# GRIPS-code/pyLBL

Measured on AMD Instinct MI355X. Metric: line×gridpoint Voigt evals/sec (whole job; per GPU: evals_per_s_per_gpu; spectra/sec: spectra_per_s), higher is better.
Workload: dtype f64; 1 GPU; BASELINE config 'target': 1 level(s) per GPU, H2O+CO2, grid 1-5000 cm-1 at 0.001 cm-1 (5000000 points), cut_off 25, remove_pedestal=False; levels_total=1, atmosphere=surface, output=gas, parallelism=levels sharded

## Files before the change

include/lbl_amd.h:

```cpp
#ifndef LBL_AMD_H_
#define LBL_AMD_H_

#include <stdint.h>

#ifdef __cplusplus
extern "C" {
#endif

#define LBL_OK              0
#define LBL_ERROR           1
#define LBL_BAD_ARGUMENT    2
#define LBL_NO_DEVICE       3
#define LBL_OUT_OF_RANGE    4
#define LBL_TABLE_OPEN_FAILED       10
#define LBL_TABLE_NO_ALIAS          11
#define LBL_TABLE_NO_TIPS           12
#define LBL_TABLE_NOT_RECTANGULAR   13
#define LBL_TABLE_NO_ISOTOPOLOGUES  14
#define LBL_TABLE_NO_TRANSITIONS    15

#define LBL_RANGE_REFERENCE 0
#define LBL_RANGE_SKIP      1

#define LBL_PREP_DEVICE     0
// ... 214 lines not shown
                     int32_t flags, double *out, int64_t level_stride);

int lbl_xsec_bands(lbl_engine *engine, int32_t xsec, double temperature, double pressure,
                   double *values);

int lbl_absorption(double pressure, double temperature, double volume_mixing_ratio,
                   int v0, int vn, int n_per_v, double *k, char *database, char *formula,
                   int cut_off, int remove_pedestal);

#ifndef LBL_NO_REFERENCE_SYMBOL
int absorption(double pressure, double temperature, double volume_mixing_ratio,
               int v0, int vn, int n_per_v, double *k, char *database, char *formula,
               int cut_off, int remove_pedestal);
#endif

typedef struct lbl_table lbl_table;
int lbl_table_read(const char *path, const char *name, lbl_table **table);
int lbl_table_shape(const lbl_table *table, int64_t *n_lines, int32_t *molecule_id,
                    int32_t *n_isotopologues, int32_t *num_iso, int32_t *num_t,
                    char *formula, int32_t formula_bytes);
int lbl_table_copy(const lbl_table *table, double *columns, int32_t *local_iso_id,
                   int64_t *isoid, double *mass, double *tips_temperature, double *tips_data);
int lbl_table_free(lbl_table *table);

int lbl_molecule_load_sqlite(lbl_engine *engine, const char *path, const char *name,
                             int32_t *molecule);

int lbl_compat_state(int32_t *device, int32_t *resident);

const char *lbl_version(void);

int lbl_wing_batches(const int32_t *bounds);

#ifdef __cplusplus
}
#endif
#endif
```

pylbl_amd/csrc/accumulate.h:

```cpp
#pragma once

#include <hip/hip_runtime.h>

#include "line_prep.h"
#include "voigt_profile.h"

namespace lbl {

struct Tiling
{
    int aligned;
    int per_cell;
    int length;
    int n_tiles;
};

__host__ __device__ inline void tile_bounds(const Tiling & t, int tile, int n_per_v, int n,
                                            long long & i0, long long & i1)
{
    if (t.aligned)
    {
        const int cell = tile/t.per_cell;
        const int sub = tile - cell*t.per_cell;
        i0 = (long long)cell*n_per_v + (long long)sub*t.length;
        i1 = i0 + t.length - 1;
        const long long cell_end = (long long)(cell + 1)*n_per_v - 1;
        if (i1 > cell_end) i1 = cell_end;
    }
    else
    {
        i0 = (long long)tile*t.length;
        i1 = i0 + t.length - 1;
    }
    if (i1 > n - 1) i1 = n - 1;
}

struct alignas(32) TileSchedule
{
// ... 5 lines not shown
{
    const double v_lo = (double)v0 + (double)i0*dv;
    const double v_hi = (double)v0 + (double)i1*dv;
    return 0.5*(v_lo + v_hi);
}

#ifndef LBL_WING_GROUP
#define LBL_WING_GROUP 8
#endif
#ifndef LBL_FAR_TERMS
#define LBL_FAR_TERMS 21
#define LBL_FAR_RATIO 4.
#endif
constexpr int kFarTerms = LBL_FAR_TERMS;
constexpr double kFarRatio = LBL_FAR_RATIO;

struct alignas(16) WorkItem
{
    int tile;
    int part, parts;
    int slot;
};

struct AccumulateArgs
{
    const LineWing * wing;
    const LineCore * core;
    const TileSchedule * schedule;
    const LevelScalars * levels;
    const WorkItem * items;
    const double * far_series;
    const int * wing_bounds;
    int wing_batches;
    double * partial;
    long long partial_slots;
    double * k;
    long long level_stride;
    long long n_lines;
    Tiling tiling;
    int n_tiles;
    int n;
    int v0, n_per_v;
    double dv;
    double v0_real;
    int scale_density;
    int accumulate;
    int inner_everywhere;
#ifdef LBL_ABLATE
    int ablate;
#endif
};

#ifdef LBL_ABLATE
#define LBL_ABLATED(a, bits) (((a).ablate & (bits)) != 0)
#else
#define LBL_ABLATED(a, bits) false
#endif

}

#include "accumulate_lines.h"

namespace lbl {

__device__ __forceinline__ void share_of(int j0, int j1, int part, int parts, float inverse,
                                         int unit_shift, int & begin, int & end)
// ... 15 lines not shown
    const int level = blockIdx.y;
    const WorkItem item = a.items[blockIdx.x];
    const int tile = item.tile;
    long long first_point, last_point;
    tile_bounds(a.tiling, tile, a.n_per_v, a.n, first_point, last_point);
    const int i0 = (int)first_point, i1 = (int)last_point;
    const TileSchedule sc = a.schedule[(long long)level*a.n_tiles + tile];
    const LineWing * __restrict__ wing = a.wing + (long long)level*a.n_lines;
    const LineCore * __restrict__ core = a.core + (long long)level*a.n_lines;

    double v[P], acc[P];
    double * slab = &partial[wave][0][0];
    __shared__ InnerStage inner_stage[4];
    const double first_index = (double)(i0 + lane);
#pragma unroll
    for (int p = 0; p < P; ++p)
    {
        const double step = (first_index + (double)(p*64))*a.dv;
        v[p] = a.v0_real + step;
        acc[p] = 0.;
    }

    const int piece = item.part*4 + wave, pieces = item.parts*4;
    GeneralList g;
    int fa0, fa1, fb0, fb1, e;
    const bool clipped_in_groups = !a.inner_everywhere && !LBL_ABLATED(a, 64);
    const float inverse = 1.f/(float)pieces;
    share_of(sc.lo, sc.a1, piece, pieces, inverse, clipped_in_groups ? 3 : 0, g.begin[0], e);
    g.count[0] = e - g.begin[0];
    share_of(sc.c1, sc.c2, piece, pieces, inverse, 0, g.begin[1], e);
    g.count[1] = e - g.begin[1];
    share_of(sc.a2, sc.hi, piece, pieces, inverse, clipped_in_groups ? 3 : 0, g.begin[2], e);
    g.count[2] = e - g.begin[2];
    share_of(sc.f1, sc.c1, piece, pieces, inverse, 2, fa0, fa1);
    share_of(sc.c2, sc.f2, piece, pieces, inverse, 2, fb0, fb1);
    g.begin[3] = fa0 + ((fa1 - fa0) & ~3);
    g.count[3] = (fa1 - fa0) & 3;
    g.begin[4] = fb0 + ((fb1 - fb0) & ~3);
    g.count[4] = (fb1 - fb0) & 3;
    if (LBL_ABLATED(a, 4)) { g.count[0] = 0; g.count[2] = 0; }
    if (LBL_ABLATED(a, 8)) { g.count[3] = 0; g.count[4] = 0; }
    if (LBL_ABLATED(a, 16)) { g.count[1] = 0; }
    if (!LBL_ABLATED(a, 2))
    {
        int batches = 1;
        if (P == 4)
        {
            const int * __restrict__ wb = a.wing_bounds + level*kWingBounds;
            const int bound[kWingBounds] = {wb[0], wb[1], wb[2], wb[3]};
            batches = __builtin_amdgcn_readfirstlane(min(wing_batches(bound), a.wing_batches));
        }
        fast_ranges<P>(wing, fa0, fa1, fb0, fb1, batches, v, acc);
    }
    bool slab_in_use = false;
    if (!LBL_ABLATED(a, 1))
    {
        GeneralList walk = g;
        if (clipped_in_groups)
        {
            clipped_ranges<P>(wing, core, g.begin[0], g.count[0], g.begin[2], g.count[2], i0, i1,
                              lane, v, acc);
            walk.count[0] = walk.count[2] = 0;
        }
        general_ranges<P>(wing, core, walk, i0, i1, lane, v, acc);
        if (!LBL_ABLATED(a, 32) && a.levels[level].inner_possible != 0.)
        {
            GeneralList inner = g;
            if (!a.inner_everywhere)
            {
                inner.count[0] = inner.count[2] = inner.count[3] = inner.count[4] = 0;
            }
            slab_in_use = inner_ranges(wing, core, inner, inner_stage[wave], i0, i1, a.v0,
                                       a.n_per_v, a.dv, lane, slab, P);
        }
    }

#pragma unroll
    for (int p = 0; p < P; ++p)
    {
        partial[wave][p][lane] = slab_in_use ? partial[wave][p][lane] + acc[p] : acc[p];
    }
    __syncthreads();

    const bool add_series = a.far_series != nullptr && item.part == 0;
    const double * __restrict__ series = a.far_series +
// ... 122 lines not shown
```

pylbl_amd/csrc/accumulate_lines.h:

```cpp
#pragma once

namespace lbl {

template <int P>
__device__ __forceinline__ void fast_ranges(const LineWing * __restrict__ wing,
                                            int a0, int a1, int b0, int b1, int batches,
                                            const double (&v)[P], double (&acc)[P])
{
    const int qa = (a1 - a0) >> 2;
    const int quads = qa + ((b1 - b0) >> 2);
    int q = 0;
#if LBL_WING_GROUP == 8
    auto eight = [&](int at, WingTerm (&l)[8]) {
        const int ja = at < qa ? a0 + 4*at : b0 + 4*(at - qa);
        const int jb = (at + 1) < qa ? a0 + 4*(at + 1) : b0 + 4*(at + 1 - qa);
#pragma unroll
        for (int i = 0; i < 4; ++i)
        {
            const LineWing wa = wing[ja + i], wb = wing[jb + i];
            l[i] = WingTerm{wa.centre, wa.g2, wa.bl};
            l[4 + i] = WingTerm{wb.centre, wb.g2, wb.bl};
        }
    };
    if (P == 4 && batches > 1)
    {
        const int eights = quads >> 1;
        for (int o = 0; o < eights; )
        {
            const int stop = min(o + batches, eights);
            double num[P], den[P];
            {
                WingTerm l[8];
                eight(2*o, l);
#pragma unroll
                for (int p = 0; p < P; ++p)
                {
                    wing_eight(v[p], l, num[p], den[p]);
                }
            }
            for (++o; o < stop; ++o)
            {
                WingTerm l[8];
                eight(2*o, l);
#pragma unroll
                for (int p = 0; p < P; ++p)
                {
                    double n, t;
                    wing_eight(v[p], l, n, t);
                    num[p] = __builtin_fma(num[p], t, n*den[p]);
                    den[p] = den[p]*t;
                }
            }
#pragma unroll
            for (int p = 0; p < P; ++p)
            {
                acc[p] = __builtin_fma(num[p], rcp_newton(den[p]), acc[p]);
            }
        }
        q = 2*eights;
    }
    for (; q + 2 <= quads; q += 2)
    {
        WingTerm l[8];
        eight(q, l);
#pragma unroll
        for (int p = 0; p < P; ++p)
        {
            acc[p] = lorentz_eight(v[p], l, acc[p]);
        }
    }
#endif
    for (; q < quads; ++q)
    {
        const int j = q < qa ? a0 + 4*q : b0 + 4*(q - qa);
        const LineWing l1 = wing[j], l2 = wing[j + 1], l3 = wing[j + 2], l4 = wing[j + 3];
#pragma unroll
        for (int p = 0; p < P; ++p)
        {
            acc[p] = lorentz_four(v[p], l1.centre, l1.g2, l1.bl, l2.centre, l2.g2, l2.bl,
                                  l3.centre, l3.g2, l3.bl, l4.centre, l4.g2, l4.bl, acc[p]);
        }
    }
}

__device__ __forceinline__ unsigned row_bits(int lo, int hi, int rows)
{
    lo = max(lo, 0);
    hi = min(hi, rows - 1);
    return lo > hi ? 0u : ((2u << hi) - 1u) & ~((1u << lo) - 1u);
}

__device__ __forceinline__ unsigned rows_meeting(int a, int b, int i0, int rows)
{
    return b < a ? 0u : row_bits((a - i0) >> 6, (b - i0) >> 6, rows);
}

__device__ __forceinline__ unsigned rows_inside(int a, int b, int i0, int rows)
{
    return b < a ? 0u : row_bits((a - i0 + 63) >> 6, (b - 63 - i0) >> 6, rows);
}

template <int P>
__device__ __forceinline__ void general_line(const LineWing & l, const LineCore & c,
                                             int i0, int i1, int lane,
                                             const double (&v)[P], double (&acc)[P])
{
    const unsigned in_window = rows_meeting(l.first, l.last, i0, P);
    if (in_window == 0)
    {
        return;
    }
    const unsigned all_region_one = rows_inside(c.mid_first, c.mid_last, i0, P) &
                                    ~rows_meeting(c.hole_first, c.hole_last, i0, P);
// ... 421 lines not shown
```

pylbl_amd/csrc/compute_stages.inc:

```
namespace {

struct CallShape
{
    Molecule * m = nullptr;
    GridSpec g;
    long long n_long = 0;
    long long stride = 0;
    RangeRule rule;
    Tiling tiling;
    int farfield = 0;
    int points = 0;
};

int shape_of(lbl_engine * engine, const ComputeRequest & rq, CallShape & s)
{
    s.m = find_molecule(engine, rq.molecule);
    if (s.m == nullptr) return fail(engine, LBL_BAD_ARGUMENT, "unknown molecule handle.");
    if (rq.n_levels < 1 || rq.temperature == nullptr || rq.pressure == nullptr ||
        rq.vmr == nullptr)
    {
        return fail(engine, LBL_BAD_ARGUMENT, "need at least one level with T, P and x.");
    }
    if (rq.n_per_v < 1 || rq.vn <= rq.v0 || rq.cut_off < 0)
    {
// ... 159 lines not shown
    bool streamed;
    int pieces;
    bool with_pedestal;
    long long out_bytes;
    long long chunk;
};

void reserve_for_call(const LinesCall & c)
{
    const ComputeRequest & rq = c.rq;
    const CallShape & s = c.shape;
    const CallTraits & t = c.traits;
    Lane & lane = c.lane;
    const long long n_lines = s.m->n_lines, n_tiles = s.tiling.n_tiles, chunk = c.chunk;
    lane.level_feed.refill((size_t)chunk);
    lane.levels.reserve((size_t)chunk);
    lane.wing.reserve((size_t)(chunk*std::max(n_lines, 1ll)));
    lane.core.reserve((size_t)(chunk*std::max(n_lines, 1ll)));
    lane.schedule.reserve((size_t)(chunk*n_tiles));
    if (t.want_k && !t.out_device) lane.staging.reserve((size_t)(chunk*s.n_long));
    if (c.with_pedestal && t.out_device && t.add_into_block)
    {
        lane.raw.reserve((size_t)(chunk*s.n_long));
    }
    if (t.want_k && s.farfield)
    {
        lane.far_series.reserve((size_t)(chunk*n_tiles*kFarTerms));
    }
    if (t.want_k)
    {
        lane.partial.reserve((size_t)std::max(1ll, chunk*c.plan.partial_slots*64*s.points));
    }
    lane.wing_bounds.reserve((size_t)(chunk*kWingBounds));
    if (rq.evals != nullptr)
    {
        lane.evals.reserve(1);
        HIP_TRY(hipMemsetAsync(lane.evals.data, 0, sizeof(unsigned long long), c.stream));
    }
    if (rq.derived != nullptr) lane.derived.reserve((size_t)(std::max(n_lines, 1ll)*8));
}

void launch_far_series(lbl_engine * engine, Lane & lane, const CallShape & s, int count,
                       hipStream_t stream)
{
    const GridSpec & g = s.g;
    const int n_tiles = s.tiling.n_tiles;
    const int n_groups = (n_tiles + kFarGroup - 1)/kFarGroup;
    const long long n_lines = s.m->n_lines;
    engine->timed(kTimeSchedule, stream, [&] {
        dim3 far_grid((unsigned)(((n_groups + 7)/8)*8), (unsigned)count);
        hipLaunchKernelGGL(farfield_series_kernel, far_grid, dim3(256), 0, stream, lane.wing.data,
                           lane.schedule.data, s.m->d_column[0].data, lane.levels.data, n_lines,
                           s.tiling, n_groups, g.v0, g.n_per_v, g.n, g.dv, lane.far_series.data);
        HIP_TRY(hipGetLastError());
    }, 1);
}

void bound_inner_regions(const Molecule & m, const RangeRule & rule, LevelScalars & lv)
{
    lv.inner_possible = 1.;
    const double foreign = lv.p_atm - lv.p_partial;
    if (foreign >= 0. && lv.p_partial >= 0. && m.min_gamma_air >= 0. &&
        m.min_gamma_self >= 0. && m.n_lines > 0)
    {
        double widest = 0.;
        for (int slot = 0; slot < kMassSlots; ++slot)
// ... 30 lines not shown
        {
            return fail(c.engine, LBL_OUT_OF_RANGE,
                        "level " + std::to_string(base + l) + ": " + why);
        }
        bound_inner_regions(*c.shape.m, c.shape.rule, lv);
    }
    if (!levels_inline(c.engine, count))
    {
        lane.level_feed.upload(lane.levels.data, (size_t)count, c.stream);
    }
    return LBL_OK;
}

int inner_points_everywhere(const LevelScalars * levels, int count, const ComputeRequest & rq,
                            const CallShape & s)
{
    double reach = 0.;
    for (int l = 0; l < count; ++l)
    {
        const LevelScalars & lv = levels[l];
        const double kk = lv.core_reach;
        reach = std::max(reach, kk < 0.5 ? kk*(rq.vn + 1.)/(1. - kk) + 2.*lv.shift_max : 1.e9);
    }
    const double tile_width = (double)s.tiling.length*s.g.dv;
    return (rq.cut_off - 1. <= reach + tile_width + 1.) ? 1 : 0;
}

struct HostPrep
{
    std::vector<LineWing> wing;
    std::vector<LineCore> core;
    std::vector<double> derived;
    std::vector<int> wing_bounds;
};

void prepare_on_host(lbl_engine * engine, Lane & lane, const ComputeRequest & rq,
                     const CallShape & s, int count, hipStream_t stream, HostPrep & hp)
{
    const Molecule & m = *s.m;
    const long long n_lines = m.n_lines;
    if (n_lines > 0)
    {
        hp.wing.resize((size_t)(count*n_lines));
        hp.core.resize((size_t)(count*n_lines));
        if (rq.derived != nullptr) hp.derived.assign((size_t)(n_lines*8), 0.);
        hp.wing_bounds.assign((size_t)(count*kWingBounds), kWingBoundsFill);
        unsigned long long total = 0;
        for (int l = 0; l < count; ++l)
        {
            for (long long j = 0; j < n_lines; ++j)
            {
                const bool ok = m.iso_slot[j] >= 0 &&
                                line_accepted(s.rule, m.column[0][j], m.order[j]);
                double * d = (rq.derived != nullptr && l == 0) ? hp.derived.data() + j*8
                                                               : nullptr;
                LineWing & w = hp.wing[(size_t)(l*n_lines + j)];
                const int status = prepare_line(
                    lane.level_feed.block[l], s.g, m.column[0][j], m.column[1][j], m.column[2][j],
                    m.column[3][j], m.column[4][j], m.column[5][j], m.column[6][j],
                    std::max(m.iso_slot[j], 0), ok, w, hp.core[(size_t)(l*n_lines + j)], d);
                if (status == 1 && w.last >= w.first) total += w.last - w.first + 1;
                int bound[kWingBounds];
                wing_line_bounds(s.g, m.column[0][j], status, w,
                                 hp.core[(size_t)(l*n_lines + j)], bound);
                for (int b = 0; b < kWingBounds; ++b)
                {
                    int & least = hp.wing_bounds[(size_t)(l*kWingBounds + b)];
                    least = std::min(least, bound[b]);
                }
            }
        }
        engine->timed(kTimePrepare, stream, [&] {
            HIP_TRY(hipMemcpyAsync(lane.wing.data, hp.wing.data(),
                                   hp.wing.size()*sizeof(LineWing), hipMemcpyHostToDevice,
                                   stream));
            HIP_TRY(hipMemcpyAsync(lane.core.data, hp.core.data(),
                                   hp.core.size()*sizeof(LineCore), hipMemcpyHostToDevice,
                                   stream));
            HIP_TRY(hipMemcpyAsync(lane.wing_bounds.data, hp.wing_bounds.data(),
                                   hp.wing_bounds.size()*sizeof(int), hipMemcpyHostToDevice,
                                   stream));
        });
        HIP_TRY(hipStreamSynchronize(stream));
        if (rq.evals != nullptr) *rq.evals += (int64_t)total;
    }
    if (rq.k != nullptr)
    {
        engine->timed(kTimeSchedule, stream, [&] {
            dim3 grid((unsigned)((8ll*s.tiling.n_tiles + 255)/256), (unsigned)count);
            hipLaunchKernelGGL(schedule_kernel, grid, dim3(256), 0, stream, m.view(),
                               lane.levels.data, s.g, s.tiling, s.farfield, lane.schedule.data);
            HIP_TRY(hipGetLastError());
        });
    }
}

void launch_prologue(const LinesCall & c, int count, HostPrep & hp)
{
    lbl_engine * engine = c.engine;
    const ComputeRequest & rq = c.rq;
    const CallShape & s = c.shape;
    Lane & lane = c.lane;
    hipStream_t stream = c.stream;
    if (engine->prep == LBL_PREP_HOST)
    {
        prepare_on_host(engine, lane, rq, s, count, stream, hp);
        return;
    }
    const bool inline_levels = levels_inline(engine, count);
    InlineLevels packed;
    if (inline_levels)
    {
        std::memcpy(packed.level, lane.level_feed.block, count*sizeof(LevelScalars));
    }
    const int prepare_blocks = (int)((s.m->n_lines + 255)/256);
    const int schedule_blocks = c.traits.want_k ? (int)((8ll*s.tiling.n_tiles + 255)/256) : 0;
    HIP_TRY(hipMemsetAsync(lane.wing_bounds.data, 0x7f, (size_t)count*kWingBounds*sizeof(int),
                           stream));
    engine->timed(kTimePrepare, stream, [&] {
        dim3 grid((unsigned)std::max(prepare_blocks + schedule_blocks, 1), (unsigned)count);
        hipLaunchKernelGGL(prologue_kernel, grid, dim3(256), 0, stream, s.m->view(),
                           lane.levels.data, packed, inline_levels ? 1 : 0, s.g, s.rule, s.tiling,
                           s.farfield, prepare_blocks, lane.wing.data, lane.core.data,
                           lane.schedule.data,
                           rq.derived != nullptr ? lane.derived.data : nullptr,
                           rq.evals != nullptr ? lane.evals.data : nullptr,
                           lane.wing_bounds.data);
        HIP_TRY(hipGetLastError());
    });
}

Lane::Pass pass_of(const LinesCall & c, long long base, int count)
{
    const CallTraits & t = c.traits;
    Lane::Pass p;
    p.base = base;
    p.count = count;
    p.target = t.out_device ? c.rq.k + base*c.shape.stride : c.lane.staging.data;
    p.target_stride = t.out_device ? c.shape.stride : c.shape.n_long;
    p.sums = p.target;
    p.sums_stride = p.target_stride;
    if (c.with_pedestal && t.out_device && t.add_into_block)
    {
        p.sums = c.lane.raw.data;
        p.sums_stride = c.shape.n_long;
    }
    p.ped_stream = c.engine->overlap_pedestal ? c.lane.side : c.stream;
    p.finish_stream = c.with_pedestal ? p.ped_stream : c.stream;
    return p;
}

void start_pedestal_search(const LinesCall & c, const Lane::Pass & p)
{
    lbl_engine * engine = c.engine;
    Lane & lane = c.lane;
    if (engine->overlap_pedestal)
    {
        lane.prepared.record(c.stream);
        HIP_TRY(hipStreamWaitEvent(lane.side, lane.prepared, 0));
    }
    engine->timed(kTimePedestal, p.ped_stream, [&] {
        pedestal_find_runs(lane.pedestal, p.ped_stream, c.shape.m->view(), lane.wing.data,
                           c.shape.g, p.count, c.rq.vn - c.rq.v0, engine->scan_chain != 0,
                           engine->poison_workspace != 0);
    }, 0);
    if (engine->overlap_pedestal)
    {
        lane.runs_found.record(lane.side);
    }
}

AccumulateArgs accumulate_args(const LinesCall & c, const Lane::Pass & p)
{
    const ComputeRequest & rq = c.rq;
    const CallShape & s = c.shape;
    const GridSpec & g = s.g;
    const Lane & lane = c.lane;
    const bool add_into = c.traits.out_device && c.traits.add_into_block;
    AccumulateArgs args;
    args.wing = lane.wing.data;
    args.core = lane.core.data;
    args.schedule = lane.schedule.data;
    args.levels = lane.levels.data;
    args.items = c.plan.items.data;
    args.far_series = s.farfield ? lane.far_series.data : nullptr;
    args.wing_bounds = lane.wing_bounds.data;
    args.wing_batches = c.engine->wing_batches;
    args.partial = lane.partial.data;
    args.partial_slots = c.plan.partial_slots;
    args.level_stride = p.sums_stride;
    args.k = p.sums;
    args.n_lines = s.m->n_lines;
    args.tiling = s.tiling;
    args.n_tiles = s.tiling.n_tiles;
    args.n = g.n;
    args.v0 = g.v0;
    args.n_per_v = g.n_per_v;
    args.dv = g.dv;
    args.v0_real = (double)g.v0;
    args.scale_density = (!c.with_pedestal && (rq.flags & LBL_SCALE_DENSITY)) ? 1 : 0;
    args.accumulate = (!c.with_pedestal && add_into) ? 1 : 0;
    args.inner_everywhere = inner_points_everywhere(lane.level_feed.block, p.count, rq, s);
#ifdef LBL_ABLATE
    args.ablate = c.engine->ablate;
#endif
    return args;
}

void launch_piece(const LinesCall & c, const Lane::Pass & p, const AccumulateArgs & args,
                  int piece)
{
    const Molecule::Plan & plan = c.plan;
    hipStream_t stream = c.stream;
    const int points = c.shape.points, count = p.count;
    const int item0 = plan.item_begin[piece], item1 = plan.item_begin[piece + 1];
    const int split0 = plan.split_begin[piece], split1 = plan.split_begin[piece + 1];
    c.engine->timed(kTimeAccumulate, stream, [&] {
        if (item1 > item0)
        {
            AccumulateArgs mine = args;
// ... 165 lines not shown
```

pylbl_amd/csrc/engine.hip:

```cpp
#include <hip/hip_runtime.h>

#include <algorithm>
#include <cmath>
#include <cstdio>
#include <cstring>
#include <functional>
#include <limits>
#include <memory>
#include <mutex>
#include <numeric>
#include <string>
#include <vector>

#include "../../include/lbl_amd.h"
#include "accumulate.h"
#include "continuum.h"
#include "xsec.h"
#include "farfield.h"
#include "flux.h"
#include "instrument.h"
#include "jacobian.h"
#include "line_prep.h"
#include "path.h"
#include "pedestal.h"
#include "radiance.h"
#include "tile_schedule.h"

#include "engine_core.h"
#include "lanes_plans.inc"
#include "compute_stages.inc"
#include "compute_call.inc"

#include "delivery.inc"
#include "slot_entry.inc"

extern "C" {

const char * lbl_version(void)
{
    return "pylbl_amd 0.1 (gfx950)";
}

int lbl_wing_batches(const int32_t * bounds)
{
    if (bounds == nullptr) return 1;
    const int bound[kWingBounds] = {bounds[0], bounds[1], bounds[2], bounds[3]};
    return wing_batches(bound);
}

int lbl_engine_create(int device, lbl_engine ** engine)
{
    if (engine == nullptr) return fail(nullptr, LBL_BAD_ARGUMENT, "engine is NULL.");
    *engine = nullptr;
    int count = 0;
    if (hipGetDeviceCount(&count) != hipSuccess || count <= 0)
    {
        return fail(nullptr, LBL_NO_DEVICE,
                    "no HIP device visible: this engine has no CPU fallback.");
    }
    if (device < 0 || device >= count)
    {
        return fail(nullptr, LBL_NO_DEVICE, "device index out of range.");
    }
    try
    {
        HIP_TRY(hipSetDevice(device));
        std::unique_ptr<lbl_engine> e(new lbl_engine());
        e->device = device;
        for (int i = 0; i < kAllLanes; ++i) e->lanes[i].create(i == kSlotLane);
        e->stream = e->lanes[0].main;
        e->copy_stream.create();
        calibrate_delivery_lanes(e.get());
        e->copies_handed_over.create();
        e->taken_over.create();
        *engine = e.release();
    }
    catch (const HipFailure & f)
    {
        return fail(nullptr, LBL_NO_DEVICE, f.message);
    }
// ... 390 lines not shown
```

pylbl_amd/csrc/engine_core.h:

```cpp
#pragma once

#include "hip_owners.h"

namespace {

using namespace lbl;

thread_local std::string g_create_error;
thread_local std::string g_thread_error;
thread_local const void * g_thread_error_engine = nullptr;

struct Molecule
{
    long long n_lines = 0;
    std::vector<double> nu_row;
    bool ascending = true;
    std::vector<int> order;
    std::vector<double> column[7];
    std::vector<int> iso_slot;
    double mass[kMassSlots];
    unsigned used_slots = 0;
    struct BadRow { int row; double nu; int local_iso_id; };
    std::vector<BadRow> bad_rows;
    double max_abs_delta = 0.;
// ... 70 lines not shown
        hipStream_t finish_stream = nullptr;
    };
    struct Finish
    {
        bool pending = false;
        Pass pass;
        GridSpec g;
        int pieces = 1, flags = 0;
        long long point_begin[9] = {};
        bool streamed = false, order_writers = false, add_into = false;
        char * host = nullptr;
        long long host_pitch = 0, columns = 0;
        double * k = nullptr;
        const double * block = nullptr;
        long long out_bytes = 0;
    } finish;
    struct Write { const char * begin = nullptr; const char * end = nullptr; Event done; };
    static constexpr int kWrites = 4;
    Write writes[kWrites];
    int next_write = 0;
    bool writes_wrapped = false;
    bool used = false;
    DeviceBuffer<LineWing> wing;
    DeviceBuffer<LineCore> core;
    DeviceBuffer<TileSchedule> schedule;
    DeviceBuffer<LevelScalars> levels;
    DeviceBuffer<double> staging;
    DeviceBuffer<double> raw;
    DeviceBuffer<double> partial;
    DeviceBuffer<double> far_series;
    DeviceBuffer<double> derived;
    DeviceBuffer<unsigned long long> evals;
    DeviceBuffer<int> wing_bounds;
    PedestalWorkspace pedestal;
    PinnedFeed<LevelScalars> level_feed;

    void create(bool urgent = false)
    {
        main.create(urgent);
        side.create(true);
        for (Event * e : {&prepared, &pedestal_done, &runs_found, &queued, &handed_over,
                          &level_feed.copied})
        {
            e->create();
        }
        for (auto & e : piece_done) e.create();
        for (auto & e : piece_summed) e.create();
        for (auto & w : writes) w.done.create();
    }
    void drain()
    {
        main.drain();
        side.drain();
    }
    ~Lane() { drain(); }
    void note_write(const void * begin, long long bytes, hipStream_t stream)
    {
        Write & w = writes[next_write];
        w.begin = reinterpret_cast<const char *>(begin);
        w.end = w.begin + bytes;
        w.done.record(stream);
        next_write = (next_write + 1) % kWrites;
        if (next_write == 0) writes_wrapped = true;
    }
};

// ... 385 lines not shown
```

pylbl_amd/csrc/tile_schedule.h:

```cpp
#pragma once

#include <hip/hip_runtime.h>

#include "accumulate.h"
#include "line_prep.h"

namespace lbl {

struct LineTableView
{
    const double * nu;
    const double * sw;
    const double * gamma_air;
    const double * gamma_self;
    const double * n_air;
    const double * elower;
    const double * delta_air;
    const int * iso_slot;
    const int * row;
    const int * sorted_of_row;
    long long n_lines;
    const int * cell_first;
    double cell_base, cell_scale;
    int cell_entries;
// ... 121 lines not shown
        s.f1 = min(max(value[6], s.a1), s.c1);
        s.f2 = min(max(value[7], s.c2), s.a2);
    }
    *out = s;
}

__global__ __launch_bounds__(256) void schedule_kernel(const LineTableView table,
                                                       const LevelScalars * __restrict__ levels,
                                                       const GridSpec g, const Tiling tiling,
                                                       const int farfield,
                                                       TileSchedule * __restrict__ schedule)
{
    const int thread = blockIdx.x*blockDim.x + threadIdx.x;
    const int tile = thread >> 3;
    const int level = blockIdx.y;
    const bool active = tile < tiling.n_tiles;
    schedule_tile(table, levels[level], g, tiling, farfield, tile, thread & 7, active,
                  schedule + (long long)level*tiling.n_tiles + (active ? tile : 0));
}

constexpr int kInlineLevels = 4;
struct InlineLevels
{
    LevelScalars level[kInlineLevels];
};

__device__ __forceinline__ void prepare_block(const LineTableView & t, const LevelScalars & lv,
                                              const GridSpec & g, const RangeRule & rule,
                                              int block, int level,
                                              LineWing * __restrict__ wing,
                                              LineCore * __restrict__ core,
                                              double * __restrict__ derived,
                                              unsigned long long * __restrict__ evals,
                                              int * __restrict__ wing_bounds)
{
    const long long j = (long long)block*blockDim.x + threadIdx.x;
    unsigned long long count = 0;
    int bound[kWingBounds] = {kWingBoundsFill, kWingBoundsFill, kWingBoundsFill, kWingBoundsFill};
    if (j < t.n_lines)
    {
        LineWing w;
        LineCore c;
        const double nu = t.nu[j];
        const int slot = t.iso_slot[j];
        const bool ok = slot >= 0 && line_accepted(rule, nu, t.row[j]);
        double * d = derived != nullptr ? derived + ((long long)level*t.n_lines + j)*8 : nullptr;
        const int status = prepare_line(lv, g, nu, t.sw[j], t.gamma_air[j],
                                        t.gamma_self[j], t.n_air[j], t.elower[j],
                                        t.delta_air[j], max(slot, 0), ok, w, c, d);
        wing[(long long)level*t.n_lines + j] = w;
        core[(long long)level*t.n_lines + j] = c;
        if (status == 1 && w.last >= w.first)
        {
            count = (unsigned long long)(w.last - w.first + 1);
        }
        wing_line_bounds(g, nu, status, w, c, bound);
    }
    {
        __shared__ int block_bound[4][kWingBounds];
#pragma unroll
        for (int b = 0; b < kWingBounds; ++b)
        {
            for (int offset = 32; offset > 0; offset >>= 1)
            {
                bound[b] = min(bound[b], __shfl_down(bound[b], offset, 64));
            }
        }
        const int wave = threadIdx.x >> 6;
        if ((threadIdx.x & 63) == 0)
        {
#pragma unroll
            for (int b = 0; b < kWingBounds; ++b) block_bound[wave][b] = bound[b];
        }
        __syncthreads();
        if (threadIdx.x < kWingBounds)
        {
            const int b = threadIdx.x;
            const int least = min(min(block_bound[0][b], block_bound[1][b]),
                                  min(block_bound[2][b], block_bound[3][b]));
            if (least != kWingBoundsFill)
            {
                atomicMin(wing_bounds + (long long)level*kWingBounds + b, least);
            }
        }
    }
    if (evals != nullptr)
    {
        for (int offset = 32; offset > 0; offset >>= 1)
        {
            count += __shfl_down(count, offset, 64);
        }
        if ((threadIdx.x & 63) == 0 && count != 0)
        {
            atomicAdd(evals, count);
        }
    }
}

__global__ __launch_bounds__(256) void prologue_kernel(const LineTableView t,
                                                       LevelScalars * __restrict__ levels,
                                                       const InlineLevels inline_levels,
                                                       const int use_inline,
                                                       const GridSpec g, const RangeRule rule,
                                                       const Tiling tiling, const int farfield,
                                                       const int prepare_blocks,
                                                       LineWing * __restrict__ wing,
                                                       LineCore * __restrict__ core,
                                                       TileSchedule * __restrict__ schedule,
                                                       double * __restrict__ derived,
                                                       unsigned long long * __restrict__ evals,
                                                       int * __restrict__ wing_bounds)
{
    const int level = blockIdx.y;
    const LevelScalars & lv = use_inline ? inline_levels.level[level] : levels[level];
    if (use_inline && blockIdx.x == 0)
    {
        const double * from = reinterpret_cast<const double *>(&inline_levels.level[level]);
        double * to = reinterpret_cast<double *>(levels + level);
        for (int i = threadIdx.x; i < (int)(sizeof(LevelScalars)/8); i += blockDim.x) to[i] = from[i];
    }
    if ((int)blockIdx.x < prepare_blocks)
    {
        prepare_block(t, lv, g, rule, blockIdx.x, level, wing, core, derived, evals,
                      wing_bounds);
        return;
    }
    const int thread = (blockIdx.x - prepare_blocks)*blockDim.x + threadIdx.x;
    const int tile = thread >> 3;
    const bool active = tile < tiling.n_tiles;
    schedule_tile(t, lv, g, tiling, farfield, tile, thread & 7, active,
                  schedule + (long long)level*tiling.n_tiles + (active ? tile : 0));
}

}
```

pylbl_amd/engine.py:

```python
from ctypes import CDLL, POINTER, Structure, byref, c_char_p, c_double, c_int32, c_int64, \
                   c_void_p
import os
from pathlib import Path
import threading
import weakref

import numpy as np

from .errors import EngineError

LIBRARY_PATH = Path(__file__).resolve().parent / "liblbl_amd.so"

LBL_OK = 0
RANGE_REFERENCE, RANGE_SKIP = 0, 1
PREP_DEVICE, PREP_HOST = 0, 1
OUT_DEVICE, ASYNC, SCALE_DENSITY, ACCUMULATE, FARFIELD, DEFER_FINISH = 1, 2, 4, 8, 16, 32
RANGE_POLICIES = {"reference": RANGE_REFERENCE, "skip": RANGE_SKIP}
PATH_OPTICAL_DEPTH, PATH_TRANSMITTANCE, PATH_CUMULATIVE, PATH_FROM_LAST, PATH_CONTINUE = \
    0x100, 0x200, 0x400, 0x800, 0x1000
PATH_RADIANCE, PATH_BRIGHTNESS = 0x2000, 0x4000
PATH_FLUX_UP = 0x8000
PATH_JACOBIAN_DEPTH, PATH_JACOBIAN_LOG_DEPTH, PATH_JACOBIAN_TEMPERATURE, \
    PATH_JACOBIAN_BOUNDARY_T, PATH_JACOBIAN_BOUNDARY_E = \
    0x10000, 0x20000, 0x40000, 0x80000, 0x100000
PATH_JACOBIAN_OUTPUTS = (
    ("radiance", PATH_RADIANCE), ("optical_depth_jacobian", PATH_JACOBIAN_DEPTH),
    ("log_optical_depth_jacobian", PATH_JACOBIAN_LOG_DEPTH),
    ("temperature_jacobian", PATH_JACOBIAN_TEMPERATURE),
    ("boundary_temperature_jacobian", PATH_JACOBIAN_BOUNDARY_T),
    ("boundary_emissivity_jacobian", PATH_JACOBIAN_BOUNDARY_E))
PATH_JACOBIAN_PER_LEVEL = ("optical_depth_jacobian", "log_optical_depth_jacobian",
                           "temperature_jacobian")

EXPORTED_SYMBOLS = (
    "lbl_engine_create", "lbl_engine_destroy", "lbl_last_error", "lbl_molecule_load",
    "lbl_molecule_free", "lbl_compute", "lbl_compute_streamed", "lbl_finish_deferred",
    "lbl_deferred", "lbl_cancel_deferred", "lbl_synchronize", "lbl_set_option", "lbl_timing",
    "lbl_timing_busy",
    "lbl_stream", "lbl_order_stream_after_engine", "lbl_order_engine_after_stream",
    "lbl_device_alloc", "lbl_device_free", "lbl_copy_to_host",
    "lbl_copy_rows_to_host", "lbl_host_alloc", "lbl_host_free",
    "lbl_line_scalars", "lbl_absorption", "absorption", "lbl_compat_state", "lbl_fill_zero",
    "lbl_version", "lbl_table_read", "lbl_table_shape", "lbl_table_copy", "lbl_table_free",
    "lbl_molecule_load_sqlite",
    "lbl_continuum_load", "lbl_continuum_free", "lbl_grid_load", "lbl_grid_free",
    "lbl_continuum_compute", "lbl_continuum_compute_many", "lbl_continuum_bands",
    "lbl_xsec_load", "lbl_xsec_free", "lbl_xsec_compute", "lbl_xsec_bands",
    "lbl_wing_batches", "lbl_path_compute", "lbl_path_radiance", "lbl_path_flux",
    "lbl_path_jacobian", "lbl_path_radiance_source", "lbl_path_flux_source",
    "lbl_instrument_create", "lbl_instrument_free", "lbl_instrument_apply",
)

VMR_SELF, VMR_H2O, VMR_O2, VMR_N2, VMR_TOTAL, VMR_COUNT = 0, 1, 2, 3, 4, 5
MAX_BANDS = 8
MAX_XSEC_BANDS = 16


class BandDescriptor(Structure):
    _fields_ = [("kind", c_int32), ("size", c_int32), ("lower_bound", c_double),
                ("resolution", c_double), ("column", c_int64*4)]

_library = None


def _preload_hip_runtime():
    import importlib.util
    import os
    import sys
    from ctypes import RTLD_GLOBAL
    if "torch" in sys.modules:
        return
    try:
        spec = importlib.util.find_spec("torch")
    except (ImportError, ValueError):
        spec = None
    if spec is None or not spec.submodule_search_locations:
        return
    for location in spec.submodule_search_locations:
        candidate = os.path.join(location, "lib", "libamdhip64.so")
        if os.path.exists(candidate):
            try:
# ... 53 lines not shown
                                          c_int64, c_int64, c_int32]
    lib.lbl_host_alloc.argtypes = [c_void_p, c_int64, POINTER(c_void_p)]
    lib.lbl_host_free.argtypes = [c_void_p, c_void_p]
    lib.lbl_line_scalars.argtypes = [c_void_p, c_int32] + [c_double]*3 + [c_int32]*6 + [c_void_p]
    lib.lbl_absorption.argtypes = [c_double]*3 + [c_int32]*3 + [c_void_p, c_char_p, c_char_p,
                                  c_int32, c_int32]
    lib.absorption.argtypes = lib.lbl_absorption.argtypes
    lib.lbl_compat_state.argtypes = [i32p, i32p]
    lib.lbl_table_read.argtypes = [c_char_p, c_char_p, POINTER(c_void_p)]
    lib.lbl_table_shape.argtypes = [c_void_p, i64p, i32p, i32p, i32p, i32p, c_char_p, c_int32]
    lib.lbl_table_copy.argtypes = [c_void_p] + [c_void_p]*6
    lib.lbl_table_free.argtypes = [c_void_p]
    lib.lbl_molecule_load_sqlite.argtypes = [c_void_p, c_char_p, c_char_p, i32p]
    lib.lbl_fill_zero.argtypes = [c_void_p, c_void_p, c_int32, c_int64, c_int64, c_int32]
    lib.lbl_version.restype = c_char_p
    lib.lbl_continuum_load.argtypes = [c_void_p, c_int32, POINTER(BandDescriptor), c_void_p,
                                       c_int64, i32p]
    lib.lbl_continuum_free.argtypes = [c_void_p, c_int32]
    lib.lbl_grid_load.argtypes = [c_void_p, c_int64, c_void_p, i32p]
    lib.lbl_grid_free.argtypes = [c_void_p, c_int32]
    lib.lbl_continuum_compute.argtypes = [c_void_p, c_int32, c_int32, c_int32, c_void_p,
                                          c_void_p, c_void_p, c_int32, c_void_p, c_int64]
    lib.lbl_continuum_compute_many.argtypes = [c_void_p, c_int32, c_void_p, c_int32, c_int32,
                                               c_void_p, c_void_p, c_void_p, c_int32, c_void_p,
                                               c_int64]
    lib.lbl_continuum_bands.argtypes = [c_void_p, c_int32, c_double, c_double, c_void_p,
                                        c_void_p]
    lib.lbl_xsec_load.argtypes = [c_void_p, c_int32, c_void_p, c_void_p, c_void_p, i32p]
    lib.lbl_xsec_free.argtypes = [c_void_p, c_int32]
    lib.lbl_xsec_compute.argtypes = [c_void_p, c_int32, c_int32, c_int32, c_void_p, c_void_p,
                                     c_void_p, c_int32, c_void_p, c_int64]
    lib.lbl_xsec_bands.argtypes = [c_void_p, c_int32, c_double, c_double, c_void_p]
    lib.lbl_wing_batches.argtypes = [c_void_p]
    lib.lbl_path_compute.argtypes = [c_void_p, c_void_p, c_int64, c_int64, c_int32, c_int32,
                                     c_int32, c_int32, c_void_p, c_int32, c_void_p, c_void_p,
                                     c_void_p, c_void_p, c_int32]
    lib.lbl_path_radiance.argtypes = [c_void_p, c_void_p, c_int64, c_int64, c_int32, c_int32,
                                      c_int32, c_int32, c_int32, c_void_p, c_void_p, c_void_p,
                                      c_void_p, c_int32, c_void_p, c_void_p, c_void_p, c_void_p,
                                      c_int32]
    lib.lbl_path_jacobian.argtypes = [c_void_p, c_void_p, c_int64, c_int64, c_int32, c_int32,
                                      c_int32, c_int32, c_int32, c_void_p, c_void_p, c_void_p,
                                      c_void_p, c_int32, c_void_p, c_void_p, c_void_p, c_void_p,
                                      c_void_p, c_void_p, c_void_p, c_void_p, c_int32]
    lib.lbl_path_flux.argtypes = [c_void_p, c_void_p, c_int64, c_int64, c_int32, c_int32, c_int32,
                                  c_int32, c_int32, c_int32, c_void_p, c_void_p, c_void_p,
                                  c_void_p, c_void_p, c_int32, c_void_p, c_void_p, c_void_p,
                                  c_void_p, c_void_p, c_void_p, c_int32]
    lib.lbl_path_radiance_source.argtypes = lib.lbl_path_radiance.argtypes[:11] + [c_void_p] + \
        lib.lbl_path_radiance.argtypes[11:]
    lib.lbl_path_flux_source.argtypes = lib.lbl_path_flux.argtypes[:13] + [c_void_p] + \
        lib.lbl_path_flux.argtypes[13:]
    lib.lbl_instrument_create.argtypes = [c_void_p, c_int32, c_int32, c_int32, c_void_p, c_void_p,
                                          c_void_p, c_int32, c_void_p, c_void_p, c_int32, i32p]
    lib.lbl_instrument_free.argtypes = [c_void_p, c_int32]
    lib.lbl_instrument_apply.argtypes = [c_void_p, c_void_p, c_int64, c_int32, c_int32, c_int32,
                                         c_void_p]
    for name in EXPORTED_SYMBOLS:
        if name not in ("lbl_last_error", "lbl_stream", "lbl_version"):
            getattr(lib, name).restype = c_int32
    _library = lib
    return lib


def _f64(array):
    return np.ascontiguousarray(array, dtype=np.float64)


def _slot_levels(temperature, pressure, accumulate, asynchronous):
    t, p = _f64(np.atleast_1d(temperature)), _f64(np.atleast_1d(pressure))
    return t, p, (ACCUMULATE if accumulate else 0) | (ASYNC if asynchronous else 0)


def _path_run(band_start, level_begin, rows, levels_per_path, from_last, asynchronous):
    starts = None if band_start is None else np.ascontiguousarray(band_start, dtype=np.int64)
    n_bands = 0 if starts is None else starts.size - 1
    flags = (PATH_FROM_LAST if from_last else 0) | (ASYNC if asynchronous else 0)
    end = int(level_begin) + rows
    if (end % int(levels_per_path) if from_last else int(level_begin) % int(levels_per_path)):
        flags |= PATH_CONTINUE
    return starts, n_bands, flags


def _per_row(beta, message, *values):
    rows, stride = int(beta.shape[0]), int(beta.shape[1])
    arrays = [_f64(np.atleast_1d(x)) for x in values]
    if any(x.shape != (rows,) for x in arrays):
        raise ValueError(message)
    return (rows, stride, *arrays)


def _per_path(n_paths, message, *values):
# ... 676 lines not shown
```

Measured before the change: 6352 billion evals/s.

## Precombine line wings in groups of four into rational polynomial records

During line preparation, each group of four Lorentz wing lines is merged into one precomputed rational function: a degree-6 numerator and degree-8 denominator polynomial around a group midpoint, stored as a 128-byte record, plus a grid-index guard range. In the far-wing loop, grid points outside the guard are evaluated with two Horner chains per quad, falling back to the exact per-line pair form near the centres. This replaces per-line loads and arithmetic in the dominant wing loop with uniform scalar record loads and fewer flops. In exchange it adds preparation work, extra device memory for the records, and possible loss of accuracy from polynomial expansion in f64 near the guard boundary.

```diff
diff --git a/include/lbl_amd.h b/include/lbl_amd.h
--- a/include/lbl_amd.h
+++ b/include/lbl_amd.h
@@ -270,6 +270,10 @@
 
 int lbl_wing_batches(const int32_t *bounds);
 
+int lbl_wing_quad(const double *centre, const double *g2, const double *bl, int32_t v0,
+                  int32_t n_per_v, double *record, int32_t *near);
+double lbl_wing_quad_guard(void);
+
 #ifdef __cplusplus
 }
 #endif
diff --git a/pylbl_amd/csrc/accumulate.h b/pylbl_amd/csrc/accumulate.h
--- a/pylbl_amd/csrc/accumulate.h
+++ b/pylbl_amd/csrc/accumulate.h
@@ -4,6 +4,7 @@
 
 #include "line_prep.h"
 #include "voigt_profile.h"
+#include "wing_quads.h"
 
 namespace lbl {
 
@@ -75,6 +76,8 @@
     const double * far_series;
     const int * wing_bounds;
     int wing_batches;
+    const WingQuad * quads;
+    const QuadNear * quad_near;
     double * partial;
     long long partial_slots;
     double * k;
@@ -156,25 +159,46 @@
     g.count[1] = e - g.begin[1];
     share_of(sc.a2, sc.hi, piece, pieces, inverse, clipped_in_groups ? 3 : 0, g.begin[2], e);
     g.count[2] = e - g.begin[2];
-    share_of(sc.f1, sc.c1, piece, pieces, inverse, 2, fa0, fa1);
-    share_of(sc.c2, sc.f2, piece, pieces, inverse, 2, fb0, fb1);
-    g.begin[3] = fa0 + ((fa1 - fa0) & ~3);
-    g.count[3] = (fa1 - fa0) & 3;
-    g.begin[4] = fb0 + ((fb1 - fb0) & ~3);
-    g.count[4] = (fb1 - fb0) & 3;
+    if constexpr (P == 4)
+    {
+        const int ma0 = min((sc.f1 + 3) & ~3, sc.c1), ma1 = max(sc.c1 & ~3, ma0);
+        const int mb0 = min((sc.c2 + 3) & ~3, sc.f2), mb1 = max(sc.f2 & ~3, mb0);
+        share_of(ma0, ma1, piece, pieces, inverse, 2, fa0, fa1);
+        share_of(mb0, mb1, piece, pieces, inverse, 2, fb0, fb1);
+        const bool heads = piece == 0, tails = piece + 1 == pieces;
+        g.begin[3] = heads ? sc.f1 : ma1;
+        g.count[3] = heads ? ma0 - sc.f1 : (tails ? sc.c1 - ma1 : 0);
+        g.begin[4] = heads ? sc.c2 : mb1;
+        g.count[4] = heads ? mb0 - sc.c2 : (tails ? sc.f2 - mb1 : 0);
+    }
+    else
+    {
+        share_of(sc.f1, sc.c1, piece, pieces, inverse, 2, fa0, fa1);
+        share_of(sc.c2, sc.f2, piece, pieces, inverse, 2, fb0, fb1);
+        g.begin[3] = fa0 + ((fa1 - fa0) & ~3);
+        g.count[3] = (fa1 - fa0) & 3;
+        g.begin[4] = fb0 + ((fb1 - fb0) & ~3);
+        g.count[4] = (fb1 - fb0) & 3;
+    }
     if (LBL_ABLATED(a, 4)) { g.count[0] = 0; g.count[2] = 0; }
     if (LBL_ABLATED(a, 8)) { g.count[3] = 0; g.count[4] = 0; }
     if (LBL_ABLATED(a, 16)) { g.count[1] = 0; }
     if (!LBL_ABLATED(a, 2))
     {
-        int batches = 1;
-        if (P == 4)
+        if constexpr (P == 4)
         {
             const int * __restrict__ wb = a.wing_bounds + level*kWingBounds;
             const int bound[kWingBounds] = {wb[0], wb[1], wb[2], wb[3]};
-            batches = __builtin_amdgcn_readfirstlane(min(wing_batches(bound), a.wing_batches));
-        }
-        fast_ranges<P>(wing, fa0, fa1, fb0, fb1, batches, v, acc);
+            const int batches =
+                __builtin_amdgcn_readfirstlane(min(wing_batches(bound), a.wing_batches));
+            const long long n_quads = a.n_lines >> 2;
+            fast_quads(wing, a.quads + level*n_quads, a.quad_near + level*n_quads, fa0, fa1, fb0,
+                       fb1, batches, i0, i1, v, acc);
+        }
+        else
+        {
+            fast_ranges<P>(wing, fa0, fa1, fb0, fb1, v, acc);
+        }
     }
     bool slab_in_use = false;
     if (!LBL_ABLATED(a, 1))
diff --git a/pylbl_amd/csrc/accumulate_lines.h b/pylbl_amd/csrc/accumulate_lines.h
--- a/pylbl_amd/csrc/accumulate_lines.h
+++ b/pylbl_amd/csrc/accumulate_lines.h
@@ -4,7 +4,7 @@
 
 template <int P>
 __device__ __forceinline__ void fast_ranges(const LineWing * __restrict__ wing,
-                                            int a0, int a1, int b0, int b1, int batches,
+                                            int a0, int a1, int b0, int b1,
                                             const double (&v)[P], double (&acc)[P])
 {
     const int qa = (a1 - a0) >> 2;
@@ -22,43 +22,6 @@
             l[4 + i] = WingTerm{wb.centre, wb.g2, wb.bl};
         }
     };
-    if (P == 4 && batches > 1)
-    {
-        const int eights = quads >> 1;
-        for (int o = 0; o < eights; )
-        {
-            const int stop = min(o + batches, eights);
-            double num[P], den[P];
-            {
-                WingTerm l[8];
-                eight(2*o, l);
-#pragma unroll
-                for (int p = 0; p < P; ++p)
-                {
-                    wing_eight(v[p], l, num[p], den[p]);
-                }
-            }
-            for (++o; o < stop; ++o)
-            {
-                WingTerm l[8];
-                eight(2*o, l);
-#pragma unroll
-                for (int p = 0; p < P; ++p)
-                {
-                    double n, t;
-                    wing_eight(v[p], l, n, t);
-                    num[p] = __builtin_fma(num[p], t, n*den[p]);
-                    den[p] = den[p]*t;
-                }
-            }
-#pragma unroll
-            for (int p = 0; p < P; ++p)
-            {
-                acc[p] = __builtin_fma(num[p], rcp_newton(den[p]), acc[p]);
-            }
-        }
-        q = 2*eights;
-    }
     for (; q + 2 <= quads; q += 2)
     {
         WingTerm l[8];
@@ -79,6 +42,92 @@
         {
             acc[p] = lorentz_four(v[p], l1.centre, l1.g2, l1.bl, l2.centre, l2.g2, l2.bl,
                                   l3.centre, l3.g2, l3.bl, l4.centre, l4.g2, l4.bl, acc[p]);
+        }
+    }
+}
+
+__device__ __forceinline__ void fast_quads(const LineWing * __restrict__ wing,
+                                           const WingQuad * __restrict__ quad,
+                                           const QuadNear * __restrict__ near,
+                                           int a0, int a1, int b0, int b1, int batches,
+                                           int i0, int i1,
+                                           const double (&v)[4], double (&acc)[4])
+{
+    constexpr int P = 4;
+    const int ga = __builtin_amdgcn_readfirstlane(a0 >> 2);
+    const int gb = __builtin_amdgcn_readfirstlane(b0 >> 2);
+    const int qa = __builtin_amdgcn_readfirstlane((a1 - a0) >> 2);
+    const int quads = qa + __builtin_amdgcn_readfirstlane((b1 - b0) >> 2);
+    if (quads == 0)
+    {
+        return;
+    }
+    auto group_of = [&](int at) { return at < qa ? ga + at : gb + (at - qa); };
+    int coming = group_of(0);
+    WingQuad next = quad[coming];
+    QuadNear next_near = near[coming];
+    int q = 0;
+    auto fraction = [&](double (&n)[P], double (&t)[P]) {
+        const int at = coming;
+        const WingQuad r = next;
+        const QuadNear guard = next_near;
+        ++q;
+        coming = group_of(min(q, quads - 1));
+        next = quad[coming];
+        next_near = near[coming];
+        if (__builtin_expect(guard.last < i0 || guard.first > i1, 1))
+        {
+#pragma unroll
+            for (int p = 0; p < P; ++p)
+            {
+                const double w = v[p] - r.m;
+                double top = __builtin_fma(r.n[6], w, r.n[5]);
+                double bottom = w + r.d[7];
+#pragma unroll
+                for (int k = 4; k >= 0; --k) top = __builtin_fma(top, w, r.n[k]);
+#pragma unroll
+                for (int k = 6; k >= 0; --k) bottom = __builtin_fma(bottom, w, r.d[k]);
+                n[p] = top;
+                t[p] = bottom;
+            }
+        }
+        else
+        {
+            const int j = 4*at;
+            const LineWing l1 = wing[j], l2 = wing[j + 1], l3 = wing[j + 2], l4 = wing[j + 3];
+#pragma unroll
+            for (int p = 0; p < P; ++p)
+            {
+                double n12, t12, n34, t34;
+                wing_pair(v[p], WingTerm{l1.centre, l1.g2, l1.bl},
+                          WingTerm{l2.centre, l2.g2, l2.bl}, n12, t12);
+                wing_pair(v[p], WingTerm{l3.centre, l3.g2, l3.bl},
+                          WingTerm{l4.centre, l4.g2, l4.bl}, n34, t34);
+                n[p] = __builtin_fma(n12, t34, n34*t12);
+                t[p] = t12*t34;
+            }
+        }
+    };
+    while (q < quads)
+    {
+        const int stop = min(q + 2*batches, quads);
+        double num[P], den[P];
+        fraction(num, den);
+        while (q < stop)
+        {
+            double n[P], t[P];
+            fraction(n, t);
+#pragma unroll
+            for (int p = 0; p < P; ++p)
+            {
+                num[p] = __builtin_fma(n[p], den[p], num[p]*t[p]);
+                den[p] = den[p]*t[p];
+            }
+        }
+#pragma unroll
+        for (int p = 0; p < P; ++p)
+        {
+            acc[p] = __builtin_fma(num[p], rcp_newton(den[p]), acc[p]);
         }
     }
 }
diff --git a/pylbl_amd/csrc/compute_stages.inc b/pylbl_amd/csrc/compute_stages.inc
--- a/pylbl_amd/csrc/compute_stages.inc
+++ b/pylbl_amd/csrc/compute_stages.inc
@@ -215,6 +215,8 @@
         lane.partial.reserve((size_t)std::max(1ll, chunk*c.plan.partial_slots*64*s.points));
     }
     lane.wing_bounds.reserve((size_t)(chunk*kWingBounds));
+    lane.quads.reserve((size_t)(chunk*std::max(n_lines >> 2, 1ll)));
+    lane.quad_near.reserve((size_t)(chunk*std::max(n_lines >> 2, 1ll)));
     if (rq.evals != nullptr)
     {
         lane.evals.reserve(1);
@@ -311,6 +313,8 @@
     std::vector<LineCore> core;
     std::vector<double> derived;
     std::vector<int> wing_bounds;
+    std::vector<WingQuad> quads;
+    std::vector<QuadNear> quad_near;
 };
 
 void prepare_on_host(lbl_engine * engine, Lane & lane, const ComputeRequest & rq,
@@ -324,6 +328,9 @@
         hp.core.resize((size_t)(count*n_lines));
         if (rq.derived != nullptr) hp.derived.assign((size_t)(n_lines*8), 0.);
         hp.wing_bounds.assign((size_t)(count*kWingBounds), kWingBoundsFill);
+        const long long n_quads = n_lines >> 2;
+        hp.quads.resize((size_t)(count*n_quads));
+        hp.quad_near.resize((size_t)(count*n_quads));
         unsigned long long total = 0;
         for (int l = 0; l < count; ++l)
         {
@@ -348,6 +355,18 @@
                     least = std::min(least, bound[b]);
                 }
             }
+            for (long long q = 0; q < n_quads; ++q)
+            {
+                double centre[4], g2[4], bl[4];
+                for (int i = 0; i < 4; ++i)
+                {
+                    const LineWing & w = hp.wing[(size_t)(l*n_lines + 4*q + i)];
+                    centre[i] = w.centre; g2[i] = w.g2; bl[i] = w.bl;
+                }
+                build_wing_quad(centre, g2, bl, s.g.v0, s.g.n_per_v,
+                                hp.quads[(size_t)(l*n_quads + q)],
+                                hp.quad_near[(size_t)(l*n_quads + q)]);
+            }
         }
         engine->timed(kTimePrepare, stream, [&] {
             HIP_TRY(hipMemcpyAsync(lane.wing.data, hp.wing.data(),
@@ -359,6 +378,15 @@
             HIP_TRY(hipMemcpyAsync(lane.wing_bounds.data, hp.wing_bounds.data(),
                                    hp.wing_bounds.size()*sizeof(int), hipMemcpyHostToDevice,
                                    stream));
+            if (n_quads > 0)
+            {
+                HIP_TRY(hipMemcpyAsync(lane.quads.data, hp.quads.data(),
+                                       hp.quads.size()*sizeof(WingQuad), hipMemcpyHostToDevice,
+                                       stream));
+                HIP_TRY(hipMemcpyAsync(lane.quad_near.data, hp.quad_near.data(),
+                                       hp.quad_near.size()*sizeof(QuadNear),
+                                       hipMemcpyHostToDevice, stream));
+            }
         });
         HIP_TRY(hipStreamSynchronize(stream));
         if (rq.evals != nullptr) *rq.evals += (int64_t)total;
@@ -404,7 +432,7 @@
                            lane.schedule.data,
                            rq.derived != nullptr ? lane.derived.data : nullptr,
                            rq.evals != nullptr ? lane.evals.data : nullptr,
-                           lane.wing_bounds.data);
+                           lane.wing_bounds.data, lane.quads.data, lane.quad_near.data);
         HIP_TRY(hipGetLastError());
     });
 }
@@ -465,6 +493,8 @@
     args.far_series = s.farfield ? lane.far_series.data : nullptr;
     args.wing_bounds = lane.wing_bounds.data;
     args.wing_batches = c.engine->wing_batches;
+    args.quads = lane.quads.data;
+    args.quad_near = lane.quad_near.data;
     args.partial = lane.partial.data;
     args.partial_slots = c.plan.partial_slots;
     args.level_stride = p.sums_stride;
diff --git a/pylbl_amd/csrc/engine.hip b/pylbl_amd/csrc/engine.hip
--- a/pylbl_amd/csrc/engine.hip
+++ b/pylbl_amd/csrc/engine.hip
@@ -46,6 +46,31 @@
     if (bounds == nullptr) return 1;
     const int bound[kWingBounds] = {bounds[0], bounds[1], bounds[2], bounds[3]};
     return wing_batches(bound);
+}
+
+int lbl_wing_quad(const double * centre, const double * g2, const double * bl, int32_t v0,
+                  int32_t n_per_v, double * record, int32_t * near)
+{
+    if (centre == nullptr || g2 == nullptr || bl == nullptr || record == nullptr ||
+        near == nullptr || n_per_v <= 0)
+    {
+        return LBL_BAD_ARGUMENT;
+    }
+    const double c[4] = {centre[0], centre[1], centre[2], centre[3]};
+    const double g[4] = {g2[0], g2[1], g2[2], g2[3]};
+    const double b[4] = {bl[0], bl[1], bl[2], bl[3]};
+    WingQuad quad;
+    QuadNear range;
+    build_wing_quad(c, g, b, v0, n_per_v, quad, range);
+    std::memcpy(record, &quad, sizeof(WingQuad));
+    near[0] = range.first;
+    near[1] = range.last;
+    return LBL_OK;
+}
+
+double lbl_wing_quad_guard(void)
+{
+    return kQuadGuard;
 }
 
 int lbl_engine_create(int device, lbl_engine ** engine)
diff --git a/pylbl_amd/csrc/engine_core.h b/pylbl_amd/csrc/engine_core.h
--- a/pylbl_amd/csrc/engine_core.h
+++ b/pylbl_amd/csrc/engine_core.h
@@ -126,6 +126,8 @@
     DeviceBuffer<double> derived;
     DeviceBuffer<unsigned long long> evals;
     DeviceBuffer<int> wing_bounds;
+    DeviceBuffer<WingQuad> quads;
+    DeviceBuffer<QuadNear> quad_near;
     PedestalWorkspace pedestal;
     PinnedFeed<LevelScalars> level_feed;
 
diff --git a/pylbl_amd/csrc/tile_schedule.h b/pylbl_amd/csrc/tile_schedule.h
--- a/pylbl_amd/csrc/tile_schedule.h
+++ b/pylbl_amd/csrc/tile_schedule.h
@@ -177,14 +177,17 @@
                                               LineCore * __restrict__ core,
                                               double * __restrict__ derived,
                                               unsigned long long * __restrict__ evals,
-                                              int * __restrict__ wing_bounds)
+                                              int * __restrict__ wing_bounds,
+                                              WingQuad * __restrict__ quads,
+                                              QuadNear * __restrict__ quad_near)
 {
     const long long j = (long long)block*blockDim.x + threadIdx.x;
     unsigned long long count = 0;
     int bound[kWingBounds] = {kWingBoundsFill, kWingBoundsFill, kWingBoundsFill, kWingBoundsFill};
+    LineWing w;
+    w.centre = 0.; w.g2 = 1.; w.bl = 0.;
     if (j < t.n_lines)
     {
-        LineWing w;
         LineCore c;
         const double nu = t.nu[j];
         const int slot = t.iso_slot[j];
@@ -200,6 +203,26 @@
             count = (unsigned long long)(w.last - w.first + 1);
         }
         wing_line_bounds(g, nu, status, w, c, bound);
+    }
+    {
+        const int lane = threadIdx.x & 63, leader = lane & ~3;
+        double centre[4], g2[4], bl[4];
+#pragma unroll
+        for (int i = 0; i < 4; ++i)
+        {
+            centre[i] = __shfl(w.centre, leader + i, 64);
+            g2[i] = __shfl(w.g2, leader + i, 64);
+            bl[i] = __shfl(w.bl, leader + i, 64);
+        }
+        if (lane == leader && j + 3 < t.n_lines)
+        {
+            const long long at = (long long)level*(t.n_lines >> 2) + (j >> 2);
+            WingQuad quad;
+            QuadNear near;
+            build_wing_quad(centre, g2, bl, g.v0, g.n_per_v, quad, near);
+            quads[at] = quad;
+            quad_near[at] = near;
+        }
     }
     {
         __shared__ int block_bound[4][kWingBounds];
@@ -254,7 +277,9 @@
                                                        TileSchedule * __restrict__ schedule,
                                                        double * __restrict__ derived,
                                                        unsigned long long * __restrict__ evals,
-                                                       int * __restrict__ wing_bounds)
+                                                       int * __restrict__ wing_bounds,
+                                                       WingQuad * __restrict__ quads,
+                                                       QuadNear * __restrict__ quad_near)
 {
     const int level = blockIdx.y;
     const LevelScalars & lv = use_inline ? inline_levels.level[level] : levels[level];
@@ -267,7 +292,7 @@
     if ((int)blockIdx.x < prepare_blocks)
     {
         prepare_block(t, lv, g, rule, blockIdx.x, level, wing, core, derived, evals,
-                      wing_bounds);
+                      wing_bounds, quads, quad_near);
         return;
     }
     const int thread = (blockIdx.x - prepare_blocks)*blockDim.x + threadIdx.x;
diff --git a/pylbl_amd/csrc/wing_quads.h b/pylbl_amd/csrc/wing_quads.h
--- /dev/null
+++ b/pylbl_amd/csrc/wing_quads.h
@@ -0,0 +1,79 @@
+#pragma once
+
+#include "line_prep.h"
+
+namespace lbl {
+
+constexpr double kQuadGuard = 6.;
+
+struct alignas(128) WingQuad
+{
+    double m;
+    double n[7];
+    double d[8];
+};
+static_assert(sizeof(WingQuad) == 128, "WingQuad is read by scalar loads: 128 bytes");
+
+struct alignas(8) QuadNear
+{
+    int first, last;
+};
+
+__host__ __device__ inline void build_wing_quad(const double (&centre)[4], const double (&g2)[4],
+                                                const double (&bl)[4], int v0, int n_per_v,
+                                                WingQuad & quad, QuadNear & near)
+{
+    const double lowest = fmin(fmin(centre[0], centre[1]), fmin(centre[2], centre[3]));
+    const double highest = fmax(fmax(centre[0], centre[1]), fmax(centre[2], centre[3]));
+    const double m = 0.5*(lowest + highest);
+    double c[4], s[4], reach2 = 0.;
+    for (int i = 0; i < 4; ++i)
+    {
+        const double h = centre[i] - m;
+        c[i] = h*h + g2[i];
+        s[i] = -2.*h;
+        reach2 = c[i] > reach2 || c[i] != c[i] ? c[i] : reach2;
+    }
+    const double p[5] = {c[0]*c[1], c[0]*s[1] + s[0]*c[1], (c[0] + s[0]*s[1]) + c[1],
+                         s[0] + s[1], 1.};
+    const double q[5] = {c[2]*c[3], c[2]*s[3] + s[2]*c[3], (c[2] + s[2]*s[3]) + c[3],
+                         s[2] + s[3], 1.};
+    const double a[3] = {bl[0]*c[1] + bl[1]*c[0], bl[0]*s[1] + bl[1]*s[0], bl[0] + bl[1]};
+    const double e[3] = {bl[2]*c[3] + bl[3]*c[2], bl[2]*s[3] + bl[3]*s[2], bl[2] + bl[3]};
+    quad.m = m;
+    for (int k = 0; k < 8; ++k)
+    {
+        double sum = 0.;
+        for (int i = 0; i <= 4; ++i)
+        {
+            const int j = k - i;
+            if (j >= 0 && j <= 4) sum += p[i]*q[j];
+        }
+        quad.d[k] = sum;
+    }
+    for (int k = 0; k < 7; ++k)
+    {
+        double left = 0., right = 0.;
+        for (int i = 0; i <= 2; ++i)
+        {
+            const int j = k - i;
+            if (j >= 0 && j <= 4)
+            {
+                left += a[i]*q[j];
+                right += e[i]*p[j];
+            }
+        }
+        quad.n[k] = left + right;
+    }
+    const double reach = kQuadGuard*sqrt(reach2);
+    double lo = floor(((m - reach) - (double)v0)*n_per_v);
+    double hi = ceil(((m + reach) - (double)v0)*n_per_v);
+    if (!(reach2 < 1.e300) || !(lo > -1.e9)) lo = -1.e9;
+    if (!(reach2 < 1.e300) || !(hi < 1.e9)) hi = 1.e9;
+    if (lo > 1.e9) lo = 1.e9;
+    if (hi < -1.e9) hi = -1.e9;
+    near.first = (int)lo;
+    near.last = (int)hi;
+}
+
+}
diff --git a/pylbl_amd/engine.py b/pylbl_amd/engine.py
--- a/pylbl_amd/engine.py
+++ b/pylbl_amd/engine.py
@@ -46,7 +46,8 @@
     "lbl_continuum_load", "lbl_continuum_free", "lbl_grid_load", "lbl_grid_free",
     "lbl_continuum_compute", "lbl_continuum_compute_many", "lbl_continuum_bands",
     "lbl_xsec_load", "lbl_xsec_free", "lbl_xsec_compute", "lbl_xsec_bands",
-    "lbl_wing_batches", "lbl_path_compute", "lbl_path_radiance", "lbl_path_flux",
+    "lbl_wing_batches", "lbl_wing_quad", "lbl_wing_quad_guard",
+    "lbl_path_compute", "lbl_path_radiance", "lbl_path_flux",
     "lbl_path_jacobian", "lbl_path_radiance_source", "lbl_path_flux_source",
     "lbl_instrument_create", "lbl_instrument_free", "lbl_instrument_apply",
 )
@@ -166,6 +167,9 @@
                                      c_void_p, c_int32, c_void_p, c_int64]
     lib.lbl_xsec_bands.argtypes = [c_void_p, c_int32, c_double, c_double, c_void_p]
     lib.lbl_wing_batches.argtypes = [c_void_p]
+    lib.lbl_wing_quad.argtypes = [c_void_p, c_void_p, c_void_p, c_int32, c_int32, c_void_p,
+                                  c_void_p]
+    lib.lbl_wing_quad_guard.restype = c_double
     lib.lbl_path_compute.argtypes = [c_void_p, c_void_p, c_int64, c_int64, c_int32, c_int32,
                                      c_int32, c_int32, c_void_p, c_int32, c_void_p, c_void_p,
                                      c_void_p, c_void_p, c_int32]
@@ -191,7 +195,7 @@
     lib.lbl_instrument_apply.argtypes = [c_void_p, c_void_p, c_int64, c_int32, c_int32, c_int32,
                                          c_void_p]
     for name in EXPORTED_SYMBOLS:
-        if name not in ("lbl_last_error", "lbl_stream", "lbl_version"):
+        if name not in ("lbl_last_error", "lbl_stream", "lbl_version", "lbl_wing_quad_guard"):
             getattr(lib, name).restype = c_int32
     _library = lib
     return lib
```

New measurement: 6869 billion evals/s (median of 6 runs). 8.1% higher.
